# isunLt/U2MKD

Hardware: AMD Instinct MI355X
Metric: LiDAR points/sec/node fwd+bwd (teacher+student+KD), 1/2/4/8 MI355X (higher is better)
Workload: dtype f32 (fp32 products emulated on the 16-bit matrix pipe: f16x2 forward / input gradient, bf16x3 weight gradient; fp32 accumulate)

## Files before the change

### include/u2mkd_hip.h

```cpp
#ifndef U2MKD_HIP_H
#define U2MKD_HIP_H

#include <stddef.h>
#include <stdint.h>

#ifdef __cplusplus
extern "C" {
#endif

typedef void *u2mkd_stream_t;

int u2mkd_version(void);
const char *u2mkd_last_error(void);
int u2mkd_stream_wait_stream(u2mkd_stream_t waiter, u2mkd_stream_t signaler);
void *u2mkd_mailbox_alloc(size_t bytes);
int u2mkd_mailbox_free(void *p);
int u2mkd_mailbox_post(const void *const *srcs, uint32_t is64, int32_t n, int64_t *slot, int64_t seq, u2mkd_stream_t s);

int u2mkd_hash(const int32_t *coords , int64_t n, int64_t *out , u2mkd_stream_t s);
int u2mkd_kernel_hash(const int32_t *coords , const int32_t *offsets , int64_t n,
                      int32_t k, int64_t *out , u2mkd_stream_t s);

size_t u2mkd_hash_table_bytes(int64_t n_refs);
int u2mkd_hash_table_build(const int64_t *refs, int64_t n_refs, void *table, u2mkd_stream_t s);
// ... 62 lines not shown
int u2mkd_debug_conv_tile_pairs_stamps(const float *in, int64_t n_in, const void *wf ,
                                       const int32_t *nbr_sorted, const int32_t *order, const int32_t *items,
                                       const int32_t *n_items, int64_t n_out, int32_t k, int32_t arith, float *out,
                                       uint64_t *stamps, u2mkd_stream_t s);
int u2mkd_debug_wgrad_stamps(const float *a, const float *b, const int32_t *pairs, const int32_t *plan, int64_t n_rows,
                             int32_t k, void *workspace, uint64_t *stamps, u2mkd_stream_t s);
int u2mkd_conv_forward_pairs(const float *in, int64_t n_in, int32_t cin, const float *wt, int32_t cout,
                             const int32_t *pair_idx, const int32_t *tile_k, const int32_t *meta, int64_t capacity,
                             int32_t k, int32_t kc, float *y , u2mkd_stream_t s);
int32_t u2mkd_conv_pairs_x3_supported(int32_t cin, int32_t cout);
int u2mkd_conv_forward_pairs_x3(const float *in, int64_t n_in, int32_t cin, const void *wf, int32_t cout,
                                const int32_t *pair_idx, const int32_t *tile_k, const int32_t *meta, int64_t capacity,
                                int32_t k, float *y , u2mkd_stream_t s);
int u2mkd_linear_forward(const float *x , int64_t n, int32_t cin, const float *w , int32_t cout,
                         const float *bias , int32_t kc, float *y, u2mkd_stream_t s);
int u2mkd_linear_forward_x3(const float *x , int64_t n, int32_t cin, const void *wf, int32_t cout,
                            const float *bias , float *y , u2mkd_stream_t s);
int32_t u2mkd_conv_pairs_f16x2_supported(int32_t cin, int32_t cout);
int u2mkd_conv_forward_pairs_f16x2(const float *in, int64_t n_in, int32_t cin, const void *wf, int32_t cout,
                                    const int32_t *pair_idx, const int32_t *tile_k, const int32_t *meta, int64_t capacity,
                                    int32_t k, float *y, u2mkd_stream_t s);
int u2mkd_linear_forward_f16x2(const float *x, int64_t n, int32_t cin, const void *wf, int32_t cout, const float *bias,
                               float *y, u2mkd_stream_t s);
int u2mkd_pairs_gather_sum(const float *y, const int32_t *pos , int64_t n_rows, int32_t k, int32_t cout,
                           float *out , u2mkd_stream_t s);
int u2mkd_kmap_rowmask(const int32_t *nbr , int64_t n_out, int32_t k, int32_t *mask ,
                       u2mkd_stream_t s);
int u2mkd_conv_forward_tiles_bf16(const void *in , int64_t n_in, int32_t cin, const void *wf, int32_t cout,
                                  const int32_t *nbr_sorted, const int32_t *order, const int32_t *items,
                                  const int32_t *n_items, int64_t n_out, int32_t k, int32_t kflip,
                                  void *out , u2mkd_stream_t s);
int u2mkd_conv_wgrad_pairs_bf16(const void *a , int32_t ca, const void *b , int32_t cb,
                                const int32_t *pairs, const int32_t *plan, int64_t n_rows, int32_t k, int32_t swap,
                                void *workspace, size_t workspace_bytes, float *dw , u2mkd_stream_t s);
int u2mkd_conv_forward_pairs_bf16(const void *in , int64_t n_in, int32_t cin, const void *wf, int32_t cout,
                                   const int32_t *pair_idx, const int32_t *tile_k, const int32_t *meta, int64_t capacity,
                                   int32_t k, void *y , u2mkd_stream_t s);
int u2mkd_linear_forward_bf16(const void *x , int64_t n, int32_t cin, const void *wf, int32_t cout,
                              const float *bias , void *y , u2mkd_stream_t s);
int u2mkd_pairs_gather_sum_bf16(const void *y , const int32_t *pos , int64_t n_rows, int32_t k,
                                int32_t cout, void *out , u2mkd_stream_t s);
size_t u2mkd_tile_schedule_workspace_bytes(int64_t n_rows);
int u2mkd_tile_schedule(const int32_t *mask , const int32_t *order , int64_t n_rows,
                        int32_t k, int32_t split0, int32_t split1, void *workspace, int32_t *tile_order,
                        int32_t *items, int32_t *n_items, u2mkd_stream_t s);
int32_t u2mkd_wgrad_plan_ints(int32_t k);
// ... 328 lines not shown
```

### u2mkd_amd/_lib.py

```python
from __future__ import annotations

import ctypes as C
import os

import torch

_HERE = os.path.dirname(os.path.abspath(__file__))
LIB_PATH = os.path.join(_HERE, 'lib', 'libu2mkd_hip%s.so' % os.environ.get('U2MKD_LIB_SUFFIX', ''))

_i32, _i64, _sz, _f32, _p = C.c_int32, C.c_int64, C.c_size_t, C.c_float, C.c_void_p

SIGNATURES = {
    'u2mkd_version': (C.c_int, []),
    'u2mkd_last_error': (C.c_char_p, []),
    'u2mkd_hash': (C.c_int, [_p, _i64, _p, _p]),
    'u2mkd_kernel_hash': (C.c_int, [_p, _p, _i64, _i32, _p, _p]),
    'u2mkd_hash_table_bytes': (_sz, [_i64]),
    'u2mkd_hash_table_build': (C.c_int, [_p, _i64, _p, _p]),
    'u2mkd_hash_table_query': (C.c_int, [_p, _i64, _p, _i64, _p, _p]),
    'u2mkd_hash_table_query2': (C.c_int, [_p, _i64, _p, _i64, _p, _p, _p]),
    'u2mkd_kmap_build_table': (C.c_int, [_p, _i64, _p, _i64, _p, _i32, _p, _p]),
    'u2mkd_kmap_invert': (C.c_int, [_p, _i64, _i32, _i64, _p, _p]),
    'u2mkd_kmap_sizes': (C.c_int, [_p, _i64, _i32, _p, _p, _p]),
    'u2mkd_kmap_compact': (C.c_int, [_p, _i64, _i32, _p, _p, _p, _p]),
# ... 21 lines not shown
    'u2mkd_pairs_gather_sum_ep': (C.c_int, [_p, _p, _i64, _i32, _i32, _p, _p, _p, _i32, _p, _p]),
    'u2mkd_pairs_gather_sum_stats_slab_rows': (_i32, []),
    'u2mkd_pairs_gather_sum_stats_supported': (_i32, [_i32]),
    'u2mkd_pairs_gather_sum_stats': (C.c_int, [_p, _p, _i64, _i32, _i32, _p, _p, _p]),
    'u2mkd_debug_conv_tile_pairs_stamps': (C.c_int, [_p, _i64, _p, _p, _p, _p, _p, _i64, _i32, _i32, _p, _p, _p]),
    'u2mkd_debug_wgrad_stamps': (C.c_int, [_p, _p, _p, _p, _i64, _i32, _p, _p, _p]),
    'u2mkd_conv_forward_pairs': (C.c_int, [_p, _i64, _i32, _p, _i32, _p, _p, _p, _i64, _i32, _i32, _p, _p]),
    'u2mkd_conv_pairs_x3_supported': (_i32, [_i32, _i32]),
    'u2mkd_conv_forward_pairs_x3': (C.c_int, [_p, _i64, _i32, _p, _i32, _p, _p, _p, _i64, _i32, _p, _p]),
    'u2mkd_linear_forward': (C.c_int, [_p, _i64, _i32, _p, _i32, _p, _i32, _p, _p]),
    'u2mkd_bn2d_workspace_bytes': (C.c_size_t, [_i64, _i32, _i64]),
    'u2mkd_bn2d_train_forward': (C.c_int, [_p, _p, _i64, _i32, _i64, _p, _p, C.c_float, C.c_float, _i32, _p, _p, _p, _p, _p, _p, _p, _p]),
    'u2mkd_bn2d_eval_forward': (C.c_int, [_p, _p, _i64, _i32, _i64, _p, _p, C.c_float, _i32, _p, _p, _p, _p]),
    'u2mkd_bn2d_backward': (C.c_int, [_p, _p, _p, _i64, _i32, _i64, _p, _p, _p, _p, _i32, _i32, _p, _p, _p, _p, _p, _p]),
    'u2mkd_bn2d_local_stats': (C.c_int, [_p, _i64, _i32, _i64, _p, _p, _p]),
    'u2mkd_bn2d_apply': (C.c_int, [_p, _p, _i64, _i32, _i64, _p, _p, _p, _p, _i32, _p, _p]),
    'u2mkd_bn2d_backward_local': (C.c_int, [_p, _p, _p, _i64, _i32, _i64, _p, _p, _p, _p, _i32, _p, _p, _p]),
    'u2mkd_bn2d_backward_local_keep': (C.c_int, [_p, _p, _p, _i64, _i32, _i64, _p, _p, _p, _p, _i32, _p, _p, _p, _p]),
    'u2mkd_bn2d_backward_apply': (C.c_int, [_p, _p, _p, _i64, _i32, _i64, _p, _p, _p, _p, _p, _i32, _p, _p, _p, _p]),
    'u2mkd_linear_forward_x3': (C.c_int, [_p, _i64, _i32, _p, _i32, _p, _p, _p]),
    'u2mkd_conv_pairs_f16x2_supported': (_i32, [_i32, _i32]),
    'u2mkd_conv_forward_pairs_f16x2': (C.c_int, [_p, _i64, _i32, _p, _i32, _p, _p, _p, _i64, _i32, _p, _p]),
    'u2mkd_linear_forward_f16x2': (C.c_int, [_p, _i64, _i32, _p, _i32, _p, _p, _p]),
    'u2mkd_pairs_capacity': (_i64, [_i64, _i64, _i32]),
    'u2mkd_pairs_build': (C.c_int, [_p, _i64, _i64, _i32, _p, _p, _p, _p, _p, _p, _p, _p, _p]),
    'u2mkd_pairs_gather_sum': (C.c_int, [_p, _p, _i64, _i32, _i32, _p, _p]),
    'u2mkd_kmap_rowmask': (C.c_int, [_p, _i64, _i32, _p, _p]),
    'u2mkd_tile_schedule_workspace_bytes': (_sz, [_i64]),
    'u2mkd_tile_schedule': (C.c_int, [_p, _p, _i64, _i32, _i32, _i32, _p, _p, _p, _p, _p]),
    'u2mkd_wgrad_plan_ints': (_i32, [_i32]),
    'u2mkd_wgrad_plan': (C.c_int, [_p, _i32, _i64, _p, _p]),
    'u2mkd_conv_wgrad_pairs_workspace_bytes': (_sz, [_i64, _i32, _i32, _i32]),
    'u2mkd_conv_wgrad_pairs': (C.c_int, [_p, _i32, _p, _i32, _p, _p, _i64, _i32, _i32, _p, _sz, _p, _p]),
    'u2mkd_conv_forward_tiles_bf16': (C.c_int, [_p, _i64, _i32, _p, _i32, _p, _p, _p, _p, _i64, _i32, _i32, _p, _p]),
    'u2mkd_conv_wgrad_pairs_bf16': (C.c_int, [_p, _i32, _p, _i32, _p, _p, _i64, _i32, _i32, _p, _sz, _p, _p]),
    'u2mkd_conv_forward_pairs_bf16': (C.c_int, [_p, _i64, _i32, _p, _i32, _p, _p, _p, _i64, _i32, _p, _p]),
    'u2mkd_linear_forward_bf16': (C.c_int, [_p, _i64, _i32, _p, _i32, _p, _p, _p]),
    'u2mkd_pairs_gather_sum_bf16': (C.c_int, [_p, _p, _i64, _i32, _i32, _p, _p]),
    'u2mkd_convolution_workspace_bytes': (_sz, [_i64, _i64, _i32, _i32, _p, _i32]),
    'u2mkd_convolution_forward': (C.c_int, [_p, _i64, _i32, _p, _i64, _i32, _p, _p, _p, _i32, _i32, _p, _sz, _p]),
    'u2mkd_convolution_backward': (C.c_int, [_p, _i64, _i32, _p, _p, _i64, _i32, _p, _p, _p, _p, _i32, _i32, _p, _sz, _p]),
    'u2mkd_bn_num_slabs': (_i64, [_i64]),
    'u2mkd_bn_train_forward': (C.c_int, [_p, _i64, _i32, _p, _p, _f32, _f32, _p, _p, _i32, _p, _p, _p, _p, _p]),
    'u2mkd_bn_train_forward_counted': (C.c_int, [_p, _i64, _i32, _p, _p, _f32, _f32, _p, _p, _p, _i32, _p, _p, _p, _p, _p]),
    'u2mkd_bn_eval_forward': (C.c_int, [_p, _i64, _i32, _p, _p, _f32, _p, _p, _i32, _p, _p, _p]),
    'u2mkd_bn_train_forward_res': (C.c_int, [_p, _p, _i64, _i32, _p, _p, _f32, _f32, _p, _p, _p, _i32, _p, _p, _p, _p, _p]),
# ... 142 lines not shown
```

### u2mkd_amd/csrc/conv.hip

```cpp
#include <stdlib.h>

#include "conv_internal.h"

namespace u2mkd {

__global__ void transpose_weights_kernel(const float *__restrict__ w, int cin, int cout, float *__restrict__ wt,
                                         int64_t total) {
    int64_t t = (int64_t)blockIdx.x * blockDim.x + threadIdx.x;
    if (t >= total) return;
    int ci = (int)(t % cin);
    int64_t r = t / cin;
    int co = (int)(r % cout);
    int64_t k = r / cout;
    wt[t] = w[(k * cin + ci) * cout + co];
}

template <int WAVES, int NB, int KC>
__global__ void __launch_bounds__(64 * WAVES)
conv_os2_kernel(const float *__restrict__ in, int cin, const float *__restrict__ wt, int cout,
                const int32_t *__restrict__ nbr, const int32_t *__restrict__ order, RowRange rr_, int K, int kflip,
                float *__restrict__ out) {
    constexpr int NT = 64 * WAVES;
    constexpr int TM = 16 * WAVES, TN = 16 * NB;
    constexpr int BS = KC + 8;
// ... 1114 lines not shown
                             tile_k, meta + 1, capacity, y, as_stream(s));
    U2_REQUIRE(rc >= 0, "u2mkd_conv_forward_pairs_x3: cin=%d and cout=%d must be multiples of 32 "
               "(ask u2mkd_conv_pairs_x3_supported first)", cin, cout);
    return rc;
}

int32_t u2mkd_conv_pairs_f16x2_supported(int32_t cin, int32_t cout) {
    static const int pref = [] {
        const char *e = getenv("U2MKD_CONV_ARITH");
        return (e && (e[0] == 'b' || (e[0] == 'f' && e[1] == '3'))) ? 0 : 1;
    }();
    return (pref && conv_px3_supported(cin, cout)) ? 1 : 0;
}

int u2mkd_conv_forward_pairs_f16x2(const float *in, int64_t n_in, int32_t cin, const void *wf, int32_t cout,
                                    const int32_t *pair_idx, const int32_t *tile_k, const int32_t *meta, int64_t capacity,
                                    int32_t k, float *y, u2mkd_stream_t s) {
    if (capacity == 0) return 0;
    U2_REQUIRE(in && wf && pair_idx && tile_k && meta && y, "u2mkd_conv_forward_pairs_f16x2: null pointer");
    U2_REQUIRE(k > 0 && n_in > 0 && capacity % 64 == 0, "u2mkd_conv_forward_pairs_f16x2: the capacity must be a multiple of 64");
    int rc = launch_conv_px3("u2mkd_conv_forward_pairs_f16x2", in, cin, reinterpret_cast<const float *>(wf), cout, pair_idx,
                             tile_k, meta + 1, capacity, y, as_stream(s), false, k);
    U2_REQUIRE(rc >= 0, "u2mkd_conv_forward_pairs_f16x2: cin=%d and cout=%d must be multiples of 32", cin, cout);
    return rc;
}

int u2mkd_linear_forward_f16x2(const float *x, int64_t n, int32_t cin, const void *wf, int32_t cout, const float *bias,
                               float *y, u2mkd_stream_t s) {
    if (n == 0) return 0;
    U2_REQUIRE(x && wf && y, "u2mkd_linear_forward_f16x2: null pointer");
    U2_REQUIRE(n > 0 && n < ((int64_t)1 << 31) - 64, "u2mkd_linear_forward_f16x2: %lld rows out of range", (long long)n);
    int rc = launch_linear_px3("u2mkd_linear_forward_f16x2", x, n, cin, reinterpret_cast<const float *>(wf), cout, bias, y,
                               as_stream(s), false, true);
    U2_REQUIRE(rc >= 0, "u2mkd_linear_forward_f16x2: cin=%d and cout=%d must be multiples of 32", cin, cout);
    return rc;
}

int u2mkd_linear_forward(const float *x, int64_t n, int32_t cin, const float *w, int32_t cout, const float *bias,
                         int32_t variant, float *y, u2mkd_stream_t s) {
    if (n == 0) return 0;
    U2_REQUIRE(x && w && y, "u2mkd_linear_forward: null pointer");
    U2_REQUIRE(cin > 0 && cin % 4 == 0 && cout > 0, "u2mkd_linear_forward: cin=%d must be a positive multiple of 4", cin);
    if (variant == 0) variant = ((int64_t)cin * cout >= 16384 && cin % 64 == 0) ? 64 : 32;
    U2_REQUIRE(variant == 32 || variant == 64, "u2mkd_linear_forward: bad variant %d", variant);
    const int c16 = (cout + 15) / 16;
    const int nb = pick_nb(c16);
// ... 229 lines not shown
```

### u2mkd_amd/csrc/conv_internal.h

```cpp
#pragma once
#include "common.h"

namespace u2mkd {

typedef float f32x4 __attribute__((ext_vector_type(4)));

#ifndef U2MKD_MFMA_GFX950_K32
#define U2MKD_MFMA_GFX950_K32 0
#endif
typedef short u2_s16x8 __attribute__((ext_vector_type(8)));
typedef short u2_s16x4 __attribute__((ext_vector_type(4)));
template <int H, class V8>
__device__ __forceinline__ f32x4 mfma_bf16_k32_half(const V8 &a, const V8 &b, f32x4 c) {
    static_assert(sizeof(V8) == 16, "mfma_bf16_k32_half: 8 bf16 per lane");
    const u2_s16x8 a8 = __builtin_bit_cast(u2_s16x8, a), b8 = __builtin_bit_cast(u2_s16x8, b);
    return H == 0 ? __builtin_amdgcn_mfma_f32_16x16x16bf16_1k(a8.lo, b8.lo, c, 0, 0, 0)
                  : __builtin_amdgcn_mfma_f32_16x16x16bf16_1k(a8.hi, b8.hi, c, 0, 0, 0);
}

template <class V8>
__device__ __forceinline__ f32x4 mfma_bf16_k32(const V8 &a, const V8 &b, f32x4 c, int = 0, int = 0, int = 0) {
    static_assert(sizeof(V8) == 16, "mfma_bf16_k32: 8 bf16 per lane");
#if U2MKD_MFMA_GFX950_K32
    typedef __bf16 bf8_t __attribute__((ext_vector_type(8)));
// ... 26 lines not shown
    const u2_h16x2 lv = {(_Float16)(a - (float)hv[0]), (_Float16)(b - (float)hv[1])};
    h = __builtin_bit_cast(uint32_t, hv);
    l = __builtin_bit_cast(uint32_t, lv);
}

struct RowRange {
    int64_t ld, begin, end;
    const int32_t *tile_order;
    const float *ep_scale = nullptr, *ep_shift = nullptr, *ep_res = nullptr;
    int ep_relu = 0;
};

int launch_conv_tp(const char *who, const float *in, int cin, const float *wf, int cout, const int32_t *nbr,
                   const int32_t *order, RowRange rr, const int32_t *items, const int32_t *n_items, int k, int kflip,
                   int arith, float *out, hipStream_t st, unsigned long long *stamps = nullptr);
bool conv_tp_supported(int cin, int cout, int k);
bool conv_tp_f16x2_supported(int cin);
int conv_tp_arith(int arith);
size_t weight_fragments_bytes(int k, int rows, int cols, int arith);
int launch_weight_fragments(const float *w, int k, int rows, int cols, int transpose, int arith, float *wf, hipStream_t st);
int launch_weight_fragments_batch(const int64_t *jobs, int n_jobs, int64_t total_units, hipStream_t st);

bool conv_px3_supported(int cin, int cout);
int launch_conv_px3(const char *who, const float *in, int cin, const float *wf, int cout, const int32_t *pair_idx,
                    const int32_t *tile_k, const int32_t *n_tiles, int64_t capacity, float *y, hipStream_t st, bool b16 = false,
                    int f16x2_k = 0 );
int launch_linear_px3(const char *who, const float *in, int64_t n_rows, int cin, const float *wf, int cout,
                      const float *bias, float *y, hipStream_t st, bool b16 = false, bool f16x2 = false);

bool conv_wgrad_x3_supported(int ca, int cb, int k);
int launch_conv_wgrad_x3(const float *a, int ca, const float *b, int cb, const int32_t *pairs, const int32_t *plan,
                         int k, int swap, int g, int merge, float *slabs, hipStream_t st, bool b16);
int conv_wgrad_x3_merge(int ca, int cb);

}
```

### u2mkd_amd/csrc/conv_px3.hip

```cpp
#include <stdlib.h>

#include <type_traits>

#include "conv_internal.h"

namespace u2mkd {

typedef __bf16 px_bf16x8 __attribute__((ext_vector_type(8)));
typedef __bf16 px_bf16x4 __attribute__((ext_vector_type(4)));

__device__ __forceinline__ void px_split3(float x, __bf16 &h, __bf16 &m, __bf16 &l) {
    h = (__bf16)x;
    float r1 = x - (float)h;
    m = (__bf16)r1;
    float r2 = r1 - (float)m;
    l = (__bf16)r2;
}

__device__ __forceinline__ px_bf16x8 px_bf8(const float4 &x) {
    f32x4 v = (f32x4){x.x, x.y, x.z, x.w};
    return __builtin_bit_cast(px_bf16x8, v);
}

template <int CTRL>
__device__ __forceinline__ float px_dpp(float v) {
    return __int_as_float(__builtin_amdgcn_update_dpp(0, __float_as_int(v), CTRL, 0xf, 0xf, true));
}

template <int NW, int NBW, bool DENSE = false, bool B16 = false, int SC = 32, int TL = 1, bool F2 = false>
__global__ void __launch_bounds__(64 * NW)
conv_px3_kernel(const float *__restrict__ in, int cin, const float *__restrict__ wf, int cout,
                const int32_t *__restrict__ pair_idx, const int32_t *__restrict__ tile_k,
                const int32_t *__restrict__ n_tiles, float *__restrict__ y, const float *__restrict__ bias = nullptr,
                int n_rows = 0, int k_total = 1) {
    static_assert(B16 ? (SC == 32 || SC == 64) : SC == 32, "step width");
    static_assert(!(F2 && B16), "f16x2 is an arithmetic of fp32 rows");
    constexpr int NT = 64 * NW, TN = 16 * NW * NBW;
    constexpr int RS = 192;
    constexpr int CH = B16 ? SC / 8 : 8;
    constexpr int RU = 64 * TL, RB = 4 * TL;
    constexpr int NCH = RU * CH;
    constexpr int LPT = (NCH + NT - 1) / NT;
    constexpr int NWF = B16 ? SC / 32 : F2 ? 2 : 3;
    const float wsc = F2 ? reinterpret_cast<const float *>(reinterpret_cast<const char *>(wf) + (size_t)k_total * cin * cout * 4)[1] : 1.f;
    const int esz = B16 ? 2 : 4;
    extern __shared__ __attribute__((aligned(16))) char smem[];
    const int tid = threadIdx.x, lane = tid & 63, wave = tid >> 6;
    const int r = lane & 15, q = lane >> 4;
    const int ntile64 = DENSE ? (n_rows + 63) / 64 : *n_tiles;
    const int ntile = (ntile64 + TL - 1) / TL;
    const int gy = (cout + TN - 1) / TN;
    const int lin = (int)blockIdx.x, wpx = (int)gridDim.x >> 3;
    int upb = wpx;
    while ((upb & 1) == 0 && ((ntile + upb - 1) / upb) * gy < 24 * (wpx / upb)) upb >>= 1;
    const int teams = 8 * (wpx / upb);
    const int team = (lin & 7) + 8 * ((lin >> 3) / upb), slot = (lin >> 3) % upb;
    if (slot >= ntile) return;
    const int gmax = (ntile - 1 - slot) / upb;
// ... 107 lines not shown
    auto adv = [&](int &t, int &s) __attribute__((always_inline)) {
        if (++s == ns) { s = 0; ++t; }
    };

    {
        int ix0[LPT];
        load_idx(tg, ix0);
        issue_G(ix0, sg, g[0]);
        issue_B(tile_offset(tw), cbw_of(tw), sw, bw[0]);
        adv(tg, sg);
        adv(tw, sw);
        load_idx(tg, ix0);
        issue_G(ix0, sg, g[1]);
        adv(tg, sg);
        load_idx(tg, gix);
        kw = tile_offset(tw);
        cw = cbw_of(tw);
        store_G(g[0], 0);
        lds_barrier();
    }

    auto step = [&](auto U, int i) __attribute__((always_inline)) {
        constexpr int u = decltype(U)::value;
        const int kcur = __builtin_amdgcn_readfirstlane(kw);
        issue_B(kcur, __builtin_amdgcn_readfirstlane(cw), sw, bw[u ^ 1]);
        issue_G(gix, sg, g[u]);
        adv(tw, sw);
        adv(tg, sg);
        kw = tile_offset(tw);
        cw = cbw_of(tw);
        load_idx(tg, gix);
        float4 a[2][NWF];
        read_frag(u, 0, a[0]);
#pragma unroll
        for (int rb = 0; rb < RB; ++rb) {
            if (rb < RB - 1) read_frag(u, rb + 1, a[(rb + 1) & 1]);
            if (B16) {
#pragma unroll
                for (int n = 0; n < NBW; ++n) {
                    f32x4 c = acc[rb][n];
#pragma unroll
                    for (int p = 0; p < NWF; ++p)
                        c = mfma_bf16_k32(px_bf8(bw[u][NWF * n + p]), px_bf8(a[rb & 1][p]), c, 0, 0, 0);
                    acc[rb][n] = c;
                }
                continue;
// ... 17 lines not shown
#pragma unroll
                for (int n = 0; n < NBW; ++n) {
                    acc[rb][n][0] = fmaf(c[n][0], osc, acc[rb][n][0]);
                    acc[rb][n][1] = fmaf(c[n][1], osc, acc[rb][n][1]);
                    acc[rb][n][2] = fmaf(c[n][2], osc, acc[rb][n][2]);
                    acc[rb][n][3] = fmaf(c[n][3], osc, acc[rb][n][3]);
                }
                continue;
            }
            const px_bf16x8 xh = px_bf8(a[rb & 1][0]), xm = px_bf8(a[rb & 1][NWF / 2]), xl = px_bf8(a[rb & 1][NWF - 1]);
#pragma unroll
            for (int n = 0; n < NBW; ++n) {
                const px_bf16x8 wh = px_bf8(bw[u][NWF * n]), wm = px_bf8(bw[u][NWF * n + NWF / 2]), wl = px_bf8(bw[u][NWF * n + NWF - 1]);
                f32x4 c = acc[rb][n];
                c = mfma_bf16_k32(wl, xh, c, 0, 0, 0);
                c = mfma_bf16_k32(wh, xl, c, 0, 0, 0);
                c = mfma_bf16_k32(wm, xm, c, 0, 0, 0);
                c = mfma_bf16_k32(wm, xh, c, 0, 0, 0);
                c = mfma_bf16_k32(wh, xm, c, 0, 0, 0);
                c = mfma_bf16_k32(wh, xh, c, 0, 0, 0);
                acc[rb][n] = c;
            }
        }
        if (sc + 1 == ns) {
            const int cbw = cbw_of(tc);
#pragma unroll
            for (int rb = 0; rb < RB; ++rb)
#pragma unroll
                for (int n = 0; n < NBW; ++n) {
                    const int col = 16 * (cbw + n) + 4 * q;
                    const int row = unit_of(tc) * RU + 16 * rb + r;
                    if (cbw + n < ncb && (!DENSE || row < n_rows)) {
                        f32x4 o = acc[rb][n];
                        if (DENSE && bias) o += *reinterpret_cast<const f32x4 *>(bias + col);
                        if (B16) {
                            px_bf16x4 ob;
                            ob[0] = (__bf16)o[0]; ob[1] = (__bf16)o[1]; ob[2] = (__bf16)o[2]; ob[3] = (__bf16)o[3];
                            *reinterpret_cast<px_bf16x4 *>(reinterpret_cast<char *>(y) + ((size_t)row * cout + col) * 2) = ob;
                        } else {
                            *reinterpret_cast<f32x4 *>(y + (size_t)row * cout + col) = o;
                        }
                    }
                    acc[rb][n] = (f32x4){0.f, 0.f, 0.f, 0.f};
                }
        }
        adv(tc, sc);
        store_G(g[u ^ 1], u ^ 1);
// ... 4 lines not shown
        step(std::integral_constant<int, 0>{}, i);
        if (i + 1 >= nsteps) break;
        step(std::integral_constant<int, 1>{}, i + 1);
    }
}

bool conv_px3_supported(int cin, int cout) { return cin >= 32 && cin % 32 == 0 && cout >= 32 && cout % 32 == 0; }

static bool px3_wide(int cout) { return cout % 256 == 0; }

static bool px3_wide3(int cout) { return cout % 192 == 0; }

struct Px3Shape { bool w3; int nbw, tl, tn; };
static Px3Shape px3_shape(int cin, int cout) {
    Px3Shape p;
    p.w3 = cout % 96 == 0 && cout % 128 != 0;
    p.tl = (cin >= 512 || cout >= 384) ? 2 : 1;
    if (p.tl == 2) p.nbw = 2;
    else p.nbw = (!p.w3 && px3_wide(cout)) || (p.w3 && px3_wide3(cout)) ? 4 : 2;
    p.tn = 16 * (p.w3 ? 3 : 4) * p.nbw;
    return p;
}

template <bool DENSE, bool B16, int SC, bool F2 = false>
static void px3_launch(const Px3Shape &p, dim3 grid, hipStream_t st, const float *in, int cin, const float *wf, int cout,
                       const int32_t *pair_idx, const int32_t *tile_k, const int32_t *n_tiles, float *y, const float *bias,
                       int n_rows, int k_total = 1) {
    const size_t lds = (size_t)2 * 64 * p.tl * 192;
#define U2_PX3(NW_, NBW_, TL_)                                                                                                  \
    hipLaunchKernelGGL((conv_px3_kernel<NW_, NBW_, DENSE, B16, SC, TL_, F2>), grid, dim3(64 * NW_), lds, st, in, cin, wf, cout, pair_idx, \
                       tile_k, n_tiles, y, bias, n_rows, k_total)
    if (p.tl == 2) {
        if (p.w3) U2_PX3(3, 2, 2); else U2_PX3(4, 2, 2);
    } else if (p.nbw == 4) {
        if (p.w3) U2_PX3(3, 4, 1); else U2_PX3(4, 4, 1);
    } else {
        if (p.w3) U2_PX3(3, 2, 1); else U2_PX3(4, 2, 1);
    }
#undef U2_PX3
}

int launch_conv_px3(const char *who, const float *in, int cin, const float *wf, int cout, const int32_t *pair_idx,
                    const int32_t *tile_k, const int32_t *n_tiles, int64_t capacity, float *y, hipStream_t st, bool b16,
                    int f16x2_k) {
    if (!conv_px3_supported(cin, cout)) return -1;
    const Px3Shape p = px3_shape(cin, cout);
    const int64_t cap_x = (p.tl == 1 && p.nbw == 2 ? 3 : 2) * 256;
    const int gy = (int)ceil_div(cout, p.tn);
    int64_t gx = std::min<int64_t>(cap_x, ceil_div(capacity / (64 * p.tl) * gy, 8) * 8);
    if (gx < 8) gx = 8;
    dim3 grid((unsigned)gx);
    if (f16x2_k > 0) px3_launch<false, false, 32, true>(p, grid, st, in, cin, wf, cout, pair_idx, tile_k, n_tiles, y, nullptr, 0, f16x2_k);
    else if (!b16) px3_launch<false, false, 32>(p, grid, st, in, cin, wf, cout, pair_idx, tile_k, n_tiles, y, nullptr, 0);
    else if (cin % 64 == 0) px3_launch<false, true, 64>(p, grid, st, in, cin, wf, cout, pair_idx, tile_k, n_tiles, y, nullptr, 0);
    else px3_launch<false, true, 32>(p, grid, st, in, cin, wf, cout, pair_idx, tile_k, n_tiles, y, nullptr, 0);
    return check_launch(who);
}

int launch_linear_px3(const char *who, const float *in, int64_t n_rows, int cin, const float *wf, int cout,
                      const float *bias, float *y, hipStream_t st, bool b16, bool f16x2) {
    if (!conv_px3_supported(cin, cout)) return -1;
    const Px3Shape p = px3_shape(cin, cout);
    const int gy = (int)ceil_div(cout, p.tn);
    const int64_t cap_x = (p.tl == 1 && p.nbw == 2 ? 3 : 2) * 256;
    int64_t gx = std::min<int64_t>(cap_x, ceil_div(ceil_div(n_rows, 64 * p.tl) * gy, 8) * 8);
    if (gx < 8) gx = 8;
    dim3 grid((unsigned)gx);
    if (f16x2) px3_launch<true, false, 32, true>(p, grid, st, in, cin, wf, cout, nullptr, nullptr, nullptr, y, bias, (int)n_rows, 1);
    else if (!b16) px3_launch<true, false, 32>(p, grid, st, in, cin, wf, cout, nullptr, nullptr, nullptr, y, bias, (int)n_rows);
    else if (cin % 64 == 0) px3_launch<true, true, 64>(p, grid, st, in, cin, wf, cout, nullptr, nullptr, nullptr, y, bias, (int)n_rows);
    else px3_launch<true, true, 32>(p, grid, st, in, cin, wf, cout, nullptr, nullptr, nullptr, y, bias, (int)n_rows);
    return check_launch(who);
}

}
// ... 1 lines not shown
```

### u2mkd_amd/torchsparse/nn/functional.py

```python
from __future__ import annotations

import os
import threading

import weakref

import torch
from torch.autograd import Function

from ... import _host
from ... import _lib as L
from ..tensor import SparseTensor
from ..utils import make_ntuple
from .utils import get_kernel_offsets

_HOST = False


def host_ops():
    global _HOST
    if _HOST is False:
        _HOST = _host.ops()
    return _HOST

# ... 431 lines not shown
        elif self._outer:
            st.extend(flags)
        return False


def _range_flag(device):
    key = (device.index, torch.cuda.current_stream(device).cuda_stream)
    f = _RANGE_FLAGS.get(key)
    if f is None:
        f = _RANGE_FLAGS[key] = torch.zeros(1, dtype=torch.int32, device=device)
    return f


def _pairs_mode(cin, cout, n_rows=0):
    env = os.environ.get('U2MKD_CONV_SCHEDULE')
    if env in ('tiles', 'pairs'):
        return env == 'pairs'
    if cout % 4:
        return False
    return cin * cout > 8192 or (cin * cout == 8192 and n_rows < 24000)


_PAIRS_X3 = os.environ.get('U2MKD_PAIRS_X3', '1') != '0'

_SCRATCH = {}


def _scratch(nbytes, device):
    key = (device.type, device.index, torch.cuda.current_stream(device).cuda_stream)
    buf = _SCRATCH.get(key)
    if buf is None or buf.numel() < nbytes:
        buf = torch.empty(int(nbytes * 1.25) + 4096, dtype=torch.uint8, device=device)
        _SCRATCH[key] = buf
    return buf


_TILE_SPLIT = tuple(int(v) for v in os.environ.get('U2MKD_TILE_SPLIT', '30,60').split(','))


class TileSchedule:

    def __init__(self, tbl):
        self.k, self.n = tbl.shape
        k, n = tbl.shape
        dev = tbl.device
        mask = torch.empty(n, dtype=torch.int32, device=dev)
# ... 47 lines not shown
        self.partial = self.slab_rows = self.of = None

    def describes(self, x):
        return self.partial is not None and self.of == (x.data_ptr(), x.shape[0], x.shape[1]) and x.dtype == torch.float32


BN_STATS_SINK = [None]
_CONV_BN_STATS = os.environ.get('U2MKD_CONV_BN_STATS', '0') != '0'


def conv_bn_stats_enabled():
    return _CONV_BN_STATS


_STATS_MAX_ROWS, _STATS_MIN_COUT = (int(v) for v in os.environ.get('U2MKD_CONV_BN_STATS_SHAPES', '100000000,8').split(','))


def _stats_in_store(n_rows, cout):
    return n_rows <= _STATS_MAX_ROWS and cout >= _STATS_MIN_COUT and bool(L.load().u2mkd_pairs_gather_sum_stats_supported(cout))


class PairSchedule:

    def __init__(self, nbr, n_in):
        k, n_out = nbr.shape
        dev = nbr.device
        lib = L.load()
        self.k, self.n_in, self.n_out = k, n_in, n_out
        self.cap = int(lib.u2mkd_pairs_capacity(n_in, n_out, k))
        nblocks = max((n_out + 1023) // 1024, 1)
        zeros = torch.zeros(k + 2, dtype=torch.int32, device=dev)
        nbsizes = zeros[:k]
        block_counts = torch.empty(k, nblocks, dtype=torch.int32, device=dev)
        self.pair_in = torch.empty(self.cap, dtype=torch.int32, device=dev)
        self.pair_out = torch.empty(self.cap, dtype=torch.int32, device=dev)
        self.pos_out = torch.empty(n_out, k, dtype=torch.int32, device=dev)
        self.pos_in = torch.full((n_in, k), -1, dtype=torch.int32, device=dev)
        self.tile_k = torch.empty(self.cap // 64, dtype=torch.int32, device=dev)
        self.meta = zeros[k:]
        if n_out and n_in:
            st = L.stream()
            L.call('u2mkd_kmap_sizes', L.ptr(nbr), n_out, k, L.ptr(nbsizes), L.ptr(block_counts), st)
            L.call('u2mkd_pairs_build', L.ptr(nbr), n_out, n_in, k, L.ptr(nbsizes), L.ptr(block_counts),
                   L.ptr(self.pair_in), L.ptr(self.pair_out), L.ptr(self.pos_out), L.ptr(self.pos_in),
                   L.ptr(self.tile_k), L.ptr(self.meta), st)
        self.nbsizes = nbsizes

    def run(self, feats, wt, cout, swap, out, variant=0, fragments=False, epilogue=None):
        n, cin = feats.shape
        st = L.stream()
        idx, pos, n_rows = (self.pair_out, self.pos_in, self.n_in) if swap else (self.pair_in, self.pos_out, self.n_out)
        if n_rows == 0:
            return out
        y = _scratch(self.cap * cout * 4, feats.device)
        if feats.dtype == torch.bfloat16:
            L.call('u2mkd_conv_forward_pairs_bf16', L.ptr(feats), n, cin, L.ptr(wt), cout, L.ptr(idx), L.ptr(self.tile_k),
                   L.ptr(self.meta), self.cap, self.k, L.ptr(y), st)
            L.call('u2mkd_pairs_gather_sum_bf16', L.ptr(y), L.ptr(pos), n_rows, self.k, cout, L.ptr(out), st)
            return out
        if fragments:
            L.call('u2mkd_conv_forward_pairs_f16x2' if fragments == 2 else 'u2mkd_conv_forward_pairs_x3', L.ptr(feats), n, cin, L.ptr(wt), cout, L.ptr(idx), L.ptr(self.tile_k),
                   L.ptr(self.meta), self.cap, self.k, L.ptr(y), st)
        else:
            L.call('u2mkd_conv_forward_pairs', L.ptr(feats), n, cin, L.ptr(wt), cout, L.ptr(idx), L.ptr(self.tile_k),
                   L.ptr(self.meta), self.cap, self.k, variant, L.ptr(y), st)
        if epilogue is not None:
            sc, sh, res, relu = epilogue
            L.call('u2mkd_pairs_gather_sum_ep', L.ptr(y), L.ptr(pos), n_rows, self.k, cout, L.ptr(sc), L.ptr(sh), L.ptr(res), int(relu),
                   L.ptr(out), st)
            return out
        sink = BN_STATS_SINK[0]
        if sink is not None and sink.partial is None and out.dtype == torch.float32 and _stats_in_store(n_rows, cout):
            rows = int(L.load().u2mkd_pairs_gather_sum_stats_slab_rows())
            partial = torch.empty((n_rows + rows - 1) // rows * 2 * cout, dtype=torch.float32, device=out.device)
            L.call('u2mkd_pairs_gather_sum_stats', L.ptr(y), L.ptr(pos), n_rows, self.k, cout, L.ptr(out), L.ptr(partial), st)
            sink.partial, sink.slab_rows, sink.of = partial, rows, (out.data_ptr(), n_rows, cout)
            return out
        L.call('u2mkd_pairs_gather_sum', L.ptr(y), L.ptr(pos), n_rows, self.k, cout, L.ptr(out), st)
        return out


KMAP_USES = {}


class KernelMap:

    def __init__(self, nbr, nbr_inv, n_in, n_out, symmetric, out_coords):
        self.nbr = nbr
        self.nbr_inv = nbr_inv
        self.n_in = int(n_in)
        self.n_out = int(n_out)
        self.k = int(nbr.shape[0])
        self.symmetric = bool(symmetric)
        self.out_coords = out_coords
        self._rulebook = None
        self._pairs = None
        self._sorted = {}
        self._pair_schedule = None
        self.tag = None

    def _note(self, use):
        if self.tag is not None:
            uses = KMAP_USES.get(self.tag)
            if uses is None:
                uses = KMAP_USES[self.tag] = set()
            uses.add(use)

    def prebuild(self, uses):
        for use in sorted(uses, key=repr):
            if use == 'pair_schedule':
                self.pair_schedule()
            elif use == 'pairs_plan':
                self.pairs_plan()
            elif use[0] == 'schedule' and (not use[1] or self.nbr_inv is not None):
                self.schedule(use[1])

    def sorted_table(self, inverse=False):
        return self.schedule(inverse).tiles()

    def schedule(self, inverse=False):
        hit = self._sorted.get(inverse)
        if hit is None:
            self._note(('schedule', bool(inverse)))
            hit = TileSchedule(self.nbr_inv if inverse else self.nbr)
            self._sorted[inverse] = hit
        return hit

    def pair_schedule(self):
        if self._pair_schedule is None:
            self._note('pair_schedule')
            self._pair_schedule = PairSchedule(self.nbr, self.n_in)
        return self._pair_schedule

    def pairs_plan(self):
        if self._pairs is None:
            self._note('pairs_plan')
            k, n_out = self.k, self.n_out
            dev = self.nbr.device
            nblocks = max((n_out + 1023) // 1024, 1)
            nbsizes = torch.zeros(k, dtype=torch.int32, device=dev)
            block_counts = torch.empty(k, nblocks, dtype=torch.int32, device=dev)
            cap = max(min(k * n_out, self.n_in * k), 1)
            pairs = torch.empty(cap, 2, dtype=torch.int32, device=dev)
            plan = torch.empty(L.load().u2mkd_wgrad_plan_ints(k), dtype=torch.int32, device=dev)
            if n_out:
                L.call('u2mkd_kmap_sizes', L.ptr(self.nbr), n_out, k, L.ptr(nbsizes), L.ptr(block_counts), L.stream())
                L.call('u2mkd_kmap_compact', L.ptr(self.nbr), n_out, k, L.ptr(nbsizes), L.ptr(block_counts),
                       L.ptr(pairs), L.stream())
            L.call('u2mkd_wgrad_plan', L.ptr(nbsizes), k, n_out, L.ptr(plan), L.stream())
            self._pairs = (pairs, nbsizes, plan)
        return self._pairs

    def rulebook(self):
        if self._rulebook is None:
# ... 20 lines not shown

def build_kmap(coords: torch.Tensor, tensor_stride, kernel_size, stride, out_coords=None) -> KernelMap:
    coords = _i32(coords).contiguous()
    L.require_cuda(coords)
    dev = coords.device
    n_in = coords.shape[0]
    offsets = get_kernel_offsets(kernel_size, stride=tensor_stride, device=dev)
    k = offsets.shape[0]
    table = coords_table(coords)
    strided = any(s > 1 for s in stride)
    if not strided:
        out_coords = coords
    elif out_coords is None:
        out_coords = spdownsample(coords, stride, kernel_size, tensor_stride)
    n_out = out_coords.shape[0]
    nbr = torch.empty(k, n_out, dtype=torch.int32, device=dev)
    L.call('u2mkd_kmap_build_table', L.ptr(table.buf), n_in, L.ptr(out_coords), n_out, L.ptr(offsets), k,
           L.ptr(nbr), L.stream())
    symmetric = (not strided) and (k % 2 == 1)
    nbr_inv = None
    if not symmetric:
        nbr_inv = torch.full((k, n_in), -1, dtype=torch.int32, device=dev)
        L.call('u2mkd_kmap_invert', L.ptr(nbr), n_out, k, n_in, L.ptr(nbr_inv), L.stream())
    return KernelMap(nbr, nbr_inv, n_in, n_out, symmetric, out_coords)


def prefetch_kmaps(x: SparseTensor, specs, level_coords=None, tag=None) -> None:
    coords, ts = x.coords, x.stride
    x.cmaps.setdefault(ts, coords)
    one = (1, 1, 1)
    for kernel_size, stride in specs:
        kernel_size, stride = make_ntuple(kernel_size, ndim=3), make_ntuple(stride, ndim=3)
        key = (ts, kernel_size, stride, one)
        kmap = x.kmaps.get(key)
        if kmap is None:
            nxt = None
            if level_coords is not None and stride != one:
                nxt = level_coords.get(tuple(ts[k] * stride[k] for k in range(3)))
            kmap = x.kmaps[key] = build_kmap(coords, ts, kernel_size, stride, out_coords=nxt)
            if tag is not None and _PREFETCH_PLANS and 'B' in _PREFETCH_PARTS:
                kmap.tag = (tag, key)
                kmap.prebuild(KMAP_USES.get(kmap.tag, ()))
        if stride != one:
            coords, ts = kmap.out_coords, tuple(ts[k] * stride[k] for k in range(3))
            x.cmaps.setdefault(ts, coords)


# ... 786 lines not shown
```

Before: 1.282 million.

## Store pair-conv rows directly with fused BN epilogue for non-overlapping strided kernels

When kernel size equals the stride (≤2), every input row belongs to exactly one pair, so the swapped (transposed) pair conv can write each result straight to its destination row. The gather-sum pass and the scratch buffer are skipped, and the optional scale/shift/residual/ReLU epilogue is applied inside the kernel. This removes one intermediate buffer round-trip and one kernel launch for these layers. It adds a new ROWS template variant and depends on the single-pair-per-row assumption being correct.

```diff
diff --git a/include/u2mkd_hip.h b/include/u2mkd_hip.h
--- a/include/u2mkd_hip.h
+++ b/include/u2mkd_hip.h
@@ -108,6 +108,11 @@
                                     int32_t k, float *y, u2mkd_stream_t s);
 int u2mkd_linear_forward_f16x2(const float *x, int64_t n, int32_t cin, const void *wf, int32_t cout, const float *bias,
                                float *y, u2mkd_stream_t s);
+int u2mkd_conv_forward_pairs_rows(const float *in, int64_t n_in, int32_t cin, const void *wf, int32_t cout,
+                                   const int32_t *pair_idx, const int32_t *pair_dst, const int32_t *tile_k, const int32_t *meta,
+                                   int64_t capacity, int32_t k, int32_t arith, int64_t n_rows, const float *scale ,
+                                   const float *shift , const float *res ,
+                                   int32_t relu, float *out , u2mkd_stream_t s);
 int u2mkd_pairs_gather_sum(const float *y, const int32_t *pos , int64_t n_rows, int32_t k, int32_t cout,
                            float *out , u2mkd_stream_t s);
 int u2mkd_kmap_rowmask(const int32_t *nbr , int64_t n_out, int32_t k, int32_t *mask ,
diff --git a/u2mkd_amd/_lib.py b/u2mkd_amd/_lib.py
--- a/u2mkd_amd/_lib.py
+++ b/u2mkd_amd/_lib.py
@@ -67,6 +67,7 @@
     'u2mkd_conv_pairs_f16x2_supported': (_i32, [_i32, _i32]),
     'u2mkd_conv_forward_pairs_f16x2': (C.c_int, [_p, _i64, _i32, _p, _i32, _p, _p, _p, _i64, _i32, _p, _p]),
     'u2mkd_linear_forward_f16x2': (C.c_int, [_p, _i64, _i32, _p, _i32, _p, _p, _p]),
+    'u2mkd_conv_forward_pairs_rows': (C.c_int, [_p, _i64, _i32, _p, _i32, _p, _p, _p, _p, _i64, _i32, _i32, _i64, _p, _p, _p, _i32, _p, _p]),
     'u2mkd_pairs_capacity': (_i64, [_i64, _i64, _i32]),
     'u2mkd_pairs_build': (C.c_int, [_p, _i64, _i64, _i32, _p, _p, _p, _p, _p, _p, _p, _p, _p]),
     'u2mkd_pairs_gather_sum': (C.c_int, [_p, _p, _i64, _i32, _i32, _p, _p]),
diff --git a/u2mkd_amd/csrc/conv.hip b/u2mkd_amd/csrc/conv.hip
--- a/u2mkd_amd/csrc/conv.hip
+++ b/u2mkd_amd/csrc/conv.hip
@@ -1160,6 +1160,24 @@
     int rc = launch_conv_px3("u2mkd_conv_forward_pairs_f16x2", in, cin, reinterpret_cast<const float *>(wf), cout, pair_idx,
                              tile_k, meta + 1, capacity, y, as_stream(s), false, k);
     U2_REQUIRE(rc >= 0, "u2mkd_conv_forward_pairs_f16x2: cin=%d and cout=%d must be multiples of 32", cin, cout);
+    return rc;
+}
+
+int u2mkd_conv_forward_pairs_rows(const float *in, int64_t n_in, int32_t cin, const void *wf, int32_t cout,
+                                   const int32_t *pair_idx, const int32_t *pair_dst, const int32_t *tile_k, const int32_t *meta,
+                                   int64_t capacity, int32_t k, int32_t arith, int64_t n_rows, const float *scale,
+                                   const float *shift, const float *res, int32_t relu, float *out, u2mkd_stream_t s) {
+    if (capacity == 0 || n_rows == 0) return 0;
+    U2_REQUIRE(in && wf && pair_idx && pair_dst && tile_k && meta && out, "u2mkd_conv_forward_pairs_rows: null pointer");
+    U2_REQUIRE(k > 0 && n_in > 0 && capacity % 64 == 0, "u2mkd_conv_forward_pairs_rows: the capacity must be a multiple of 64");
+    U2_REQUIRE(arith == 2 || arith == 4, "u2mkd_conv_forward_pairs_rows: arith=%d must be 2 (bf16x3) or 4 (f16x2)", arith);
+    U2_REQUIRE(n_rows > 0 && n_rows < ((int64_t)1 << 31), "u2mkd_conv_forward_pairs_rows: %lld rows out of range", (long long)n_rows);
+    U2_REQUIRE((scale == nullptr) == (shift == nullptr) && (scale || !res),
+               "u2mkd_conv_forward_pairs_rows: scale and shift come together, a residual only with them");
+    const Px3Rows rows{pair_dst, n_rows, scale, shift, res, (int)relu};
+    int rc = launch_conv_px3("u2mkd_conv_forward_pairs_rows", in, cin, reinterpret_cast<const float *>(wf), cout, pair_idx,
+                             tile_k, meta + 1, capacity, out, as_stream(s), false, arith == 4 ? k : 0, &rows);
+    U2_REQUIRE(rc >= 0, "u2mkd_conv_forward_pairs_rows: cin=%d and cout=%d must be multiples of 32", cin, cout);
     return rc;
 }
 
diff --git a/u2mkd_amd/csrc/conv_internal.h b/u2mkd_amd/csrc/conv_internal.h
--- a/u2mkd_amd/csrc/conv_internal.h
+++ b/u2mkd_amd/csrc/conv_internal.h
@@ -72,9 +72,16 @@
 int launch_weight_fragments_batch(const int64_t *jobs, int n_jobs, int64_t total_units, hipStream_t st);
 
 bool conv_px3_supported(int cin, int cout);
+struct Px3Rows {
+    const int32_t *dst_idx;
+    int64_t n_rows;
+    const float *scale, *shift, *res;
+    int relu;
+};
 int launch_conv_px3(const char *who, const float *in, int cin, const float *wf, int cout, const int32_t *pair_idx,
                     const int32_t *tile_k, const int32_t *n_tiles, int64_t capacity, float *y, hipStream_t st, bool b16 = false,
-                    int f16x2_k = 0 );
+                    int f16x2_k = 0 ,
+                    const Px3Rows *rows = nullptr);
 int launch_linear_px3(const char *who, const float *in, int64_t n_rows, int cin, const float *wf, int cout,
                       const float *bias, float *y, hipStream_t st, bool b16 = false, bool f16x2 = false);
 
diff --git a/u2mkd_amd/csrc/conv_px3.hip b/u2mkd_amd/csrc/conv_px3.hip
--- a/u2mkd_amd/csrc/conv_px3.hip
+++ b/u2mkd_amd/csrc/conv_px3.hip
@@ -27,13 +27,16 @@
     return __int_as_float(__builtin_amdgcn_update_dpp(0, __float_as_int(v), CTRL, 0xf, 0xf, true));
 }
 
-template <int NW, int NBW, bool DENSE = false, bool B16 = false, int SC = 32, int TL = 1, bool F2 = false>
+template <int NW, int NBW, bool DENSE = false, bool B16 = false, int SC = 32, int TL = 1, bool F2 = false, bool ROWS = false>
 __global__ void __launch_bounds__(64 * NW)
 conv_px3_kernel(const float *__restrict__ in, int cin, const float *__restrict__ wf, int cout,
                 const int32_t *__restrict__ pair_idx, const int32_t *__restrict__ tile_k,
                 const int32_t *__restrict__ n_tiles, float *__restrict__ y, const float *__restrict__ bias = nullptr,
-                int n_rows = 0, int k_total = 1) {
+                int n_rows = 0, int k_total = 1, const int32_t *__restrict__ dst_idx = nullptr,
+                const float *__restrict__ ep_scale = nullptr, const float *__restrict__ ep_shift = nullptr,
+                const float *__restrict__ ep_res = nullptr, int ep_relu = 0) {
     static_assert(B16 ? (SC == 32 || SC == 64) : SC == 32, "step width");
+    static_assert(!(ROWS && (DENSE || B16)), "the one-pair-per-row store is a form of the fp32 pair schedule");
     static_assert(!(F2 && B16), "f16x2 is an arithmetic of fp32 rows");
     constexpr int NT = 64 * NW, TN = 16 * NW * NBW;
     constexpr int RS = 192;
@@ -187,6 +190,12 @@
 
     auto step = [&](auto U, int i) __attribute__((always_inline)) {
         constexpr int u = decltype(U)::value;
+        int drow[RB];
+        if (ROWS) {
+            const int32_t *pd = dst_idx + (size_t)unit_of(tc) * RU + r;
+#pragma unroll
+            for (int rb = 0; rb < RB; ++rb) drow[rb] = pd[16 * rb];
+        }
         const int kcur = __builtin_amdgcn_readfirstlane(kw);
         issue_B(kcur, __builtin_amdgcn_readfirstlane(cw), sw, bw[u ^ 1]);
         issue_G(gix, sg, g[u]);
@@ -250,7 +259,45 @@
                 acc[rb][n] = c;
             }
         }
-        if (sc + 1 == ns) {
+        if (ROWS) {
+            if (sc + 1 == ns) {
+                const int cbw = cbw_of(tc);
+#pragma unroll
+                for (int n = 0; n < NBW; ++n) {
+                    const int col = 16 * (cbw + n) + 4 * q;
+                    const bool cok = cbw + n < ncb;
+                    f32x4 esc = (f32x4){1.f, 1.f, 1.f, 1.f}, esh = (f32x4){0.f, 0.f, 0.f, 0.f};
+                    if (ep_scale && cok) {
+                        esc = *reinterpret_cast<const f32x4 *>(ep_scale + col);
+                        esh = *reinterpret_cast<const f32x4 *>(ep_shift + col);
+                    }
+#pragma unroll
+                    for (int rb = 0; rb < RB; ++rb) {
+                        const int d = drow[rb];
+                        if (cok && (unsigned)d < (unsigned)n_rows) {
+                            f32x4 o;
+#pragma unroll
+                            for (int c = 0; c < 4; ++c) o[c] = 0.f + acc[rb][n][c];
+                            if (ep_scale) {
+#pragma unroll
+                                for (int c = 0; c < 4; ++c) o[c] = fmaf(o[c], esc[c], esh[c]);
+                                if (ep_res) {
+                                    const f32x4 rs = *reinterpret_cast<const f32x4 *>(ep_res + (size_t)d * cout + col);
+#pragma unroll
+                                    for (int c = 0; c < 4; ++c) o[c] += rs[c];
+                                }
+                                if (ep_relu) {
+#pragma unroll
+                                    for (int c = 0; c < 4; ++c) o[c] = fmaxf(o[c], 0.f);
+                                }
+                            }
+                            *reinterpret_cast<f32x4 *>(y + (size_t)d * cout + col) = o;
+                        }
+                        acc[rb][n] = (f32x4){0.f, 0.f, 0.f, 0.f};
+                    }
+                }
+            }
+        } else if (sc + 1 == ns) {
             const int cbw = cbw_of(tc);
 #pragma unroll
             for (int rb = 0; rb < RB; ++rb)
@@ -301,14 +348,15 @@
     return p;
 }
 
-template <bool DENSE, bool B16, int SC, bool F2 = false>
+template <bool DENSE, bool B16, int SC, bool F2 = false, bool ROWS = false>
 static void px3_launch(const Px3Shape &p, dim3 grid, hipStream_t st, const float *in, int cin, const float *wf, int cout,
                        const int32_t *pair_idx, const int32_t *tile_k, const int32_t *n_tiles, float *y, const float *bias,
-                       int n_rows, int k_total = 1) {
+                       int n_rows, int k_total = 1, const Px3Rows *rows = nullptr) {
     const size_t lds = (size_t)2 * 64 * p.tl * 192;
+    const Px3Rows rw = rows ? *rows : Px3Rows{nullptr, 0, nullptr, nullptr, nullptr, 0};
 #define U2_PX3(NW_, NBW_, TL_)                                                                                                  \
-    hipLaunchKernelGGL((conv_px3_kernel<NW_, NBW_, DENSE, B16, SC, TL_, F2>), grid, dim3(64 * NW_), lds, st, in, cin, wf, cout, pair_idx, \
-                       tile_k, n_tiles, y, bias, n_rows, k_total)
+    hipLaunchKernelGGL((conv_px3_kernel<NW_, NBW_, DENSE, B16, SC, TL_, F2, ROWS>), grid, dim3(64 * NW_), lds, st, in, cin, wf, cout, pair_idx, \
+                       tile_k, n_tiles, y, bias, n_rows, k_total, rw.dst_idx, rw.scale, rw.shift, rw.res, rw.relu)
     if (p.tl == 2) {
         if (p.w3) U2_PX3(3, 2, 2); else U2_PX3(4, 2, 2);
     } else if (p.nbw == 4) {
@@ -321,15 +369,17 @@
 
 int launch_conv_px3(const char *who, const float *in, int cin, const float *wf, int cout, const int32_t *pair_idx,
                     const int32_t *tile_k, const int32_t *n_tiles, int64_t capacity, float *y, hipStream_t st, bool b16,
-                    int f16x2_k) {
-    if (!conv_px3_supported(cin, cout)) return -1;
+                    int f16x2_k, const Px3Rows *rows) {
+    if (!conv_px3_supported(cin, cout) || (rows && b16)) return -1;
     const Px3Shape p = px3_shape(cin, cout);
     const int64_t cap_x = (p.tl == 1 && p.nbw == 2 ? 3 : 2) * 256;
     const int gy = (int)ceil_div(cout, p.tn);
     int64_t gx = std::min<int64_t>(cap_x, ceil_div(capacity / (64 * p.tl) * gy, 8) * 8);
     if (gx < 8) gx = 8;
     dim3 grid((unsigned)gx);
-    if (f16x2_k > 0) px3_launch<false, false, 32, true>(p, grid, st, in, cin, wf, cout, pair_idx, tile_k, n_tiles, y, nullptr, 0, f16x2_k);
+    if (rows && f16x2_k > 0) px3_launch<false, false, 32, true, true>(p, grid, st, in, cin, wf, cout, pair_idx, tile_k, n_tiles, y, nullptr, (int)rows->n_rows, f16x2_k, rows);
+    else if (rows) px3_launch<false, false, 32, false, true>(p, grid, st, in, cin, wf, cout, pair_idx, tile_k, n_tiles, y, nullptr, (int)rows->n_rows, 1, rows);
+    else if (f16x2_k > 0) px3_launch<false, false, 32, true>(p, grid, st, in, cin, wf, cout, pair_idx, tile_k, n_tiles, y, nullptr, 0, f16x2_k);
     else if (!b16) px3_launch<false, false, 32>(p, grid, st, in, cin, wf, cout, pair_idx, tile_k, n_tiles, y, nullptr, 0);
     else if (cin % 64 == 0) px3_launch<false, true, 64>(p, grid, st, in, cin, wf, cout, pair_idx, tile_k, n_tiles, y, nullptr, 0);
     else px3_launch<false, true, 32>(p, grid, st, in, cin, wf, cout, pair_idx, tile_k, n_tiles, y, nullptr, 0);
diff --git a/u2mkd_amd/torchsparse/nn/functional.py b/u2mkd_amd/torchsparse/nn/functional.py
--- a/u2mkd_amd/torchsparse/nn/functional.py
+++ b/u2mkd_amd/torchsparse/nn/functional.py
@@ -477,6 +477,7 @@
 
 
 _PAIRS_X3 = os.environ.get('U2MKD_PAIRS_X3', '1') != '0'
+_PAIRS_ROWS = os.environ.get('U2MKD_PAIRS_ROWS', '1') != '0'
 
 _SCRATCH = {}
 
@@ -570,11 +571,12 @@
 
 class PairSchedule:
 
-    def __init__(self, nbr, n_in):
+    def __init__(self, nbr, n_in, single_in=False):
         k, n_out = nbr.shape
         dev = nbr.device
         lib = L.load()
         self.k, self.n_in, self.n_out = k, n_in, n_out
+        self.single_in = bool(single_in)
         self.cap = int(lib.u2mkd_pairs_capacity(n_in, n_out, k))
         nblocks = max((n_out + 1023) // 1024, 1)
         zeros = torch.zeros(k + 2, dtype=torch.int32, device=dev)
@@ -599,6 +601,12 @@
         st = L.stream()
         idx, pos, n_rows = (self.pair_out, self.pos_in, self.n_in) if swap else (self.pair_in, self.pos_out, self.n_out)
         if n_rows == 0:
+            return out
+        if swap and self.single_in and _PAIRS_ROWS and fragments and feats.dtype == torch.float32 and BN_STATS_SINK[0] is None:
+            sc, sh, res, relu = epilogue if epilogue is not None else (None, None, None, False)
+            L.call('u2mkd_conv_forward_pairs_rows', L.ptr(feats), n, cin, L.ptr(wt), cout, L.ptr(idx), L.ptr(self.pair_in),
+                   L.ptr(self.tile_k), L.ptr(self.meta), self.cap, self.k, 4 if fragments == 2 else 2, n_rows, L.ptr(sc), L.ptr(sh),
+                   L.ptr(res), int(relu), L.ptr(out), st)
             return out
         y = _scratch(self.cap * cout * 4, feats.device)
         if feats.dtype == torch.bfloat16:
@@ -633,8 +641,9 @@
 
 class KernelMap:
 
-    def __init__(self, nbr, nbr_inv, n_in, n_out, symmetric, out_coords):
+    def __init__(self, nbr, nbr_inv, n_in, n_out, symmetric, out_coords, single_in=False):
         self.nbr = nbr
+        self.single_in = bool(single_in)
         self.nbr_inv = nbr_inv
         self.n_in = int(n_in)
         self.n_out = int(n_out)
@@ -677,7 +686,7 @@
     def pair_schedule(self):
         if self._pair_schedule is None:
             self._note('pair_schedule')
-            self._pair_schedule = PairSchedule(self.nbr, self.n_in)
+            self._pair_schedule = PairSchedule(self.nbr, self.n_in, single_in=self.single_in)
         return self._pair_schedule
 
     def pairs_plan(self):
@@ -744,7 +753,9 @@
     if not symmetric:
         nbr_inv = torch.full((k, n_in), -1, dtype=torch.int32, device=dev)
         L.call('u2mkd_kmap_invert', L.ptr(nbr), n_out, k, n_in, L.ptr(nbr_inv), L.stream())
-    return KernelMap(nbr, nbr_inv, n_in, n_out, symmetric, out_coords)
+    ks = make_ntuple(kernel_size, ndim=3)
+    single_in = strided and all(ks[d] == stride[d] and ks[d] <= 2 for d in range(3))
+    return KernelMap(nbr, nbr_inv, n_in, n_out, symmetric, out_coords, single_in=single_in)
 
 
 def prefetch_kmaps(x: SparseTensor, specs, level_coords=None, tag=None) -> None:
```

Measured after the change: 1.287 million, median of 4. No clear change (+0.4%).
